# lukors/kanter_core

Measured on AMD Instinct MI355X. Metric: node-Mpix/s on 4096x4096 f32x4, 32-node graph, higher is better.
Workload: dtype f32

## Files before the change

bindings/rust/kanter_core_amd_sys.rs:

```rust
#![allow(non_camel_case_types, dead_code)]
use std::os::raw::{c_char, c_void};

pub const KC_OK: i32 = 0;
pub const KC_ERR_GENERIC: i32 = 1;
pub const KC_ERR_CANCELED: i32 = 2;
pub const KC_ERR_IMAGE: i32 = 3;
pub const KC_ERR_INVALID_BUFFER_COUNT: i32 = 4;
pub const KC_ERR_INVALID_NODE_ID: i32 = 5;
pub const KC_ERR_INVALID_NODE_TYPE: i32 = 6;
pub const KC_ERR_INVALID_SLOT_ID: i32 = 7;
pub const KC_ERR_INVALID_SLOT_TYPE: i32 = 8;
pub const KC_ERR_INVALID_EDGE: i32 = 9;
pub const KC_ERR_NO_SLOT_DATA: i32 = 10;
pub const KC_ERR_SLOT_OCCUPIED: i32 = 11;
pub const KC_ERR_SLOT_NOT_OCCUPIED: i32 = 12;
pub const KC_ERR_UNABLE_TO_LOCK: i32 = 13;
pub const KC_ERR_NODE_PROCESSING: i32 = 14;
pub const KC_ERR_POISON: i32 = 15;
pub const KC_ERR_TRY_LOCK: i32 = 16;
pub const KC_ERR_NODE_DIRTY: i32 = 17;
pub const KC_ERR_IO: i32 = 18;
pub const KC_ERR_INVALID_NAME: i32 = 19;
pub const KC_ERR_HIP: i32 = 100;
pub const KC_ERR_NO_DEVICE: i32 = 101;
// ... 264 lines not shown
    pub fn kc_status_string(status: i32) -> *const c_char;
    pub fn kc_set_fusion(enabled: i32) -> i32;
    pub fn kc_get_fusion() -> i32;
    pub fn kc_set_resize_mode(mode: i32) -> i32;
    pub fn kc_get_resize_mode() -> i32;
    pub fn kc_set_cache_policy(mode: i32) -> i32;
    pub fn kc_get_cache_policy() -> i32;
    pub fn kc_set_option(name: *const c_char, value: i32) -> i32;
    pub fn kc_get_option(name: *const c_char, value: *mut i32) -> i32;
    pub fn kc_resize_upsample_plan(in_n: u32, out_n: u32, filter: i32, eligible: *mut i32, info: *mut i32, rows: *mut f32, cap: usize) -> i32;
    pub fn kc_resize_down2_plan(in_n: u32, out_n: u32, filter: i32, info: *mut i32, left_count: *mut u32, w: *mut f32, wcap: usize, vrec: *mut u32, vcap: usize, hw: *mut f32, hcap: usize) -> i32;
    pub fn kc_stats(bytes_in_use: *mut u64, bytes_cached: *mut u64, kernel_launches: *mut u64) -> i32;
    pub fn kc_stats_algorithmic_bytes(bytes: *mut u64) -> i32;
    pub fn kc_stats_counter(name: *const c_char, value: *mut u64) -> i32;
    pub fn kc_pool_trim() -> i32;
    pub fn kc_set_specialize(mode: i32, after: i32) -> i32;
    pub fn kc_get_specialize() -> i32;
    pub fn kc_specialize_wait() -> i32;
    pub fn kc_specialize_stats(kernels_compiled: *mut u64, compiles_failed: *mut u64, specialized_launches: *mut u64, compiles_pending: *mut u64) -> i32;
    pub fn kc_specialize_compile_check(words: *const u32, n_ops: u32, n_in: u32, start_src: i32, flat: i32, source: *mut c_char, cap: usize) -> i32;
    pub fn kc_specialize_compile_check_mask(words: *const u32, n_ops: u32, n_in: u32, start_src: i32, flat: i32, nt_mask: u32, source: *mut c_char, cap: usize) -> i32;
    pub fn kc_set_chain_quads(quads: i32) -> i32;
    pub fn kc_get_chain_quads() -> i32;
    pub fn kc_specialize_compile_check_upsample(words: *const u32, n_ops: u32, n_in: u32, start_src: i32, taps: u32, wide: i32, source: *mut c_char, cap: usize) -> i32;
    pub fn kc_kernel_cache_set_dir(dir: *const c_char) -> i32;
    pub fn kc_kernel_cache_stats(files_accepted: *mut u64, files_refused: *mut u64, files_written: *mut u64, kernels_loaded: *mut u64) -> i32;
    pub fn kc_kernel_cache_precompile(words: *const u32, n_ops: u32, n_in: u32, start_src: i32, flat: i32, nt_mask: u32, up_taps: u32, up_wide: i32, dir: *const c_char) -> i32;
    pub fn kc_specialize_reset() -> i32;
    pub fn kc_kernel_cache_precompile_packed(words: *const u32, n_ops: u32, n_in: u32, start_src: i32, flat: i32, nt_mask: u32, in_tiers: u32, dir: *const c_char) -> i32;
    pub fn kc_set_pack_sources(mode: i32) -> i32;
    pub fn kc_get_pack_sources() -> i32;
    pub fn kc_set_pack_budget_mb(mb: i32) -> i32;
    pub fn kc_get_pack_budget_mb() -> i32;
    pub fn kc_plane_alloc(width: u32, height: u32, out: *mut *mut KcPlane) -> i32;
    pub fn kc_plane_const(width: u32, height: u32, value: f32, out: *mut *mut KcPlane) -> i32;
    pub fn kc_plane_wrap(device_ptr: *mut c_void, width: u32, height: u32, pitch_bytes: usize, out: *mut *mut KcPlane) -> i32;
    pub fn kc_plane_retain(p: *mut KcPlane) -> i32;
    pub fn kc_plane_release(p: *mut KcPlane) -> i32;
    pub fn kc_plane_size(p: *const KcPlane, width: *mut u32, height: *mut u32) -> i32;
    pub fn kc_plane_is_const(p: *const KcPlane, is_const: *mut i32, value: *mut f32) -> i32;
    pub fn kc_plane_materialize(p: *mut KcPlane) -> i32;
    pub fn kc_plane_device_ptr(p: *mut KcPlane, device_ptr: *mut *mut c_void, pitch_bytes: *mut usize) -> i32;
    pub fn kc_plane_upload_f32(p: *mut KcPlane, host: *const f32, host_pitch_bytes: usize) -> i32;
    pub fn kc_plane_download_f32(p: *mut KcPlane, host: *mut f32, host_pitch_bytes: usize) -> i32;
    pub fn kc_image_gray(p: *mut KcPlane, out: *mut *mut KcImage) -> i32;
    pub fn kc_image_rgba(planes: *const *mut KcPlane, out: *mut *mut KcImage) -> i32;
    pub fn kc_image_retain(img: *mut KcImage) -> i32;
    pub fn kc_image_release(img: *mut KcImage) -> i32;
    pub fn kc_image_is_rgba(img: *const KcImage, is_rgba: *mut i32) -> i32;
    pub fn kc_image_size(img: *const KcImage, size: *mut KcSize) -> i32;
    pub fn kc_image_plane(img: *const KcImage, channel: i32, out: *mut *mut KcPlane) -> i32;
    pub fn kc_image_from_value(size: KcSize, value: f32, rgba: i32, out: *mut *mut KcImage) -> i32;
    pub fn kc_image_as_type(img: *const KcImage, rgba: i32, out: *mut *mut KcImage) -> i32;
    pub fn kc_image_materialize(img: *mut KcImage) -> i32;
    pub fn kc_image_from_u8(host: *const u8, width: u32, height: u32, channels: i32, out: *mut *mut KcImage) -> i32;
    pub fn kc_image_to_u8(img: *mut KcImage, srgb: i32, host_rgba8: *mut u8) -> i32;
    pub fn kc_u8_pipe_create(width: u32, height: u32, channels: i32, depth: i32, out: *mut *mut KcU8Pipe) -> i32;
    pub fn kc_u8_pipe_free(pipe: *mut KcU8Pipe) -> i32;
    pub fn kc_u8_pipe_buffers(pipe: *mut KcU8Pipe, slot: i32, host_in: *mut *mut u8, host_out: *mut *const u8) -> i32;
    pub fn kc_u8_pipe_upload(pipe: *mut KcU8Pipe, slot: i32, out: *mut *mut KcImage) -> i32;
    pub fn kc_u8_pipe_download(pipe: *mut KcU8Pipe, slot: i32, img: *mut KcImage, srgb: i32) -> i32;
    pub fn kc_u8_pipe_wait_download(pipe: *mut KcU8Pipe, slot: i32) -> i32;
    pub fn kc_image_from_f32(host_planes: *const *const f32, n_planes: i32, width: u32, height: u32, out: *mut *mut KcImage) -> i32;
    pub fn kc_image_to_f32(img: *mut KcImage, host_planes: *const *mut f32, n_planes: i32) -> i32;
    pub fn kc_device_image_validate(d: *const KcDeviceImage, extent_bytes: *mut usize) -> i32;
    pub fn kc_image_from_device(src: *const KcDeviceImage, flags: u32, hip_stream: *mut c_void, out: *mut *mut KcImage) -> i32;
// ... 129 lines not shown
```

include/kanter_core_amd.h:

```cpp
#ifndef KANTER_CORE_AMD_H
#define KANTER_CORE_AMD_H

#include <stddef.h>
#include <stdint.h>

#ifdef __cplusplus
extern "C" {
#endif

#define KC_API __attribute__((visibility("default")))

typedef enum kc_status {
    KC_OK = 0,
    KC_ERR_GENERIC = 1,
    KC_ERR_CANCELED = 2,
    KC_ERR_IMAGE = 3,
    KC_ERR_INVALID_BUFFER_COUNT = 4,
    KC_ERR_INVALID_NODE_ID = 5,
    KC_ERR_INVALID_NODE_TYPE = 6,
    KC_ERR_INVALID_SLOT_ID = 7,
    KC_ERR_INVALID_SLOT_TYPE = 8,
    KC_ERR_INVALID_EDGE = 9,
    KC_ERR_NO_SLOT_DATA = 10,
    KC_ERR_SLOT_OCCUPIED = 11,
// ... 66 lines not shown
KC_API int kc_get_option(const char *name, int *value);
KC_API int kc_resize_upsample_plan(uint32_t in_n, uint32_t out_n, int filter, int *eligible, int32_t info[5], float *rows,
                                   size_t cap);
KC_API int kc_resize_down2_plan(uint32_t in_n, uint32_t out_n, int filter, int32_t info[5], uint32_t *left_count, float *w, size_t wcap,
                                uint32_t *vrec, size_t vcap, float *hw, size_t hcap);
KC_API int kc_stats(uint64_t *bytes_in_use, uint64_t *bytes_cached, uint64_t *kernel_launches);
KC_API int kc_stats_algorithmic_bytes(uint64_t *bytes);
KC_API int kc_stats_counter(const char *name, uint64_t *value);
KC_API int kc_pool_trim(void);
KC_API int kc_set_specialize(int mode, int after);
KC_API int kc_get_specialize(void);
KC_API int kc_specialize_wait(void);
KC_API int kc_specialize_stats(uint64_t *kernels_compiled, uint64_t *compiles_failed, uint64_t *specialized_launches,
                               uint64_t *compiles_pending);
KC_API int kc_specialize_compile_check(const uint32_t *words, uint32_t n_ops, uint32_t n_in, int start_src, int flat,
                                       char *source, size_t cap);
KC_API int kc_specialize_compile_check_mask(const uint32_t *words, uint32_t n_ops, uint32_t n_in, int start_src, int flat,
                                            uint32_t nt_mask, char *source, size_t cap);
KC_API int kc_set_chain_quads(int quads);
KC_API int kc_get_chain_quads(void);
KC_API int kc_specialize_compile_check_upsample(const uint32_t *words, uint32_t n_ops, uint32_t n_in, int start_src, uint32_t taps,
                                                int wide, char *source, size_t cap);
KC_API int kc_kernel_cache_set_dir(const char *dir);
KC_API int kc_kernel_cache_stats(uint64_t *files_accepted, uint64_t *files_refused, uint64_t *files_written, uint64_t *kernels_loaded);
KC_API int kc_kernel_cache_precompile(const uint32_t *words, uint32_t n_ops, uint32_t n_in, int start_src, int flat, uint32_t nt_mask,
                                      uint32_t up_taps, int up_wide, const char *dir);
KC_API int kc_specialize_reset(void);
KC_API int kc_kernel_cache_precompile_packed(const uint32_t *words, uint32_t n_ops, uint32_t n_in, int start_src, int flat,
                                             uint32_t nt_mask, uint32_t in_tiers, const char *dir);
KC_API int kc_set_pack_sources(int mode);
KC_API int kc_get_pack_sources(void);
KC_API int kc_set_pack_budget_mb(int mb);
KC_API int kc_get_pack_budget_mb(void);

KC_API int kc_plane_alloc(uint32_t width, uint32_t height, kc_plane **out);
KC_API int kc_plane_const(uint32_t width, uint32_t height, float value, kc_plane **out);
KC_API int kc_plane_wrap(void *device_ptr, uint32_t width, uint32_t height, size_t pitch_bytes, kc_plane **out);
KC_API int kc_plane_retain(kc_plane *p);
KC_API int kc_plane_release(kc_plane *p);
KC_API int kc_plane_size(const kc_plane *p, uint32_t *width, uint32_t *height);
KC_API int kc_plane_is_const(const kc_plane *p, int *is_const, float *value);
KC_API int kc_plane_materialize(kc_plane *p);
KC_API int kc_plane_device_ptr(kc_plane *p, void **device_ptr, size_t *pitch_bytes);
KC_API int kc_plane_upload_f32(kc_plane *p, const float *host, size_t host_pitch_bytes);
KC_API int kc_plane_download_f32(kc_plane *p, float *host, size_t host_pitch_bytes);

KC_API int kc_image_gray(kc_plane *p, kc_image **out);
KC_API int kc_image_rgba(kc_plane *const planes[4], kc_image **out);
KC_API int kc_image_retain(kc_image *img);
KC_API int kc_image_release(kc_image *img);
KC_API int kc_image_is_rgba(const kc_image *img, int *is_rgba);
KC_API int kc_image_size(const kc_image *img, kc_size *size);
KC_API int kc_image_plane(const kc_image *img, int channel, kc_plane **out);
KC_API int kc_image_from_value(kc_size size, float value, int rgba, kc_image **out);
KC_API int kc_image_as_type(const kc_image *img, int rgba, kc_image **out);
KC_API int kc_image_materialize(kc_image *img);
KC_API int kc_image_from_u8(const uint8_t *host, uint32_t width, uint32_t height, int channels, kc_image **out);
KC_API int kc_image_to_u8(kc_image *img, int srgb, uint8_t *host_rgba8);
KC_API int kc_u8_pipe_create(uint32_t width, uint32_t height, int channels, int depth, kc_u8_pipe **out);
KC_API int kc_u8_pipe_free(kc_u8_pipe *pipe);
KC_API int kc_u8_pipe_buffers(kc_u8_pipe *pipe, int slot, uint8_t **host_in, const uint8_t **host_out);
KC_API int kc_u8_pipe_upload(kc_u8_pipe *pipe, int slot, kc_image **out);
KC_API int kc_u8_pipe_download(kc_u8_pipe *pipe, int slot, kc_image *img, int srgb);
KC_API int kc_u8_pipe_wait_download(kc_u8_pipe *pipe, int slot);
KC_API int kc_image_from_f32(const float *const host_planes[], int n_planes, uint32_t width, uint32_t height, kc_image **out);
KC_API int kc_image_to_f32(kc_image *img, float *const host_planes[], int n_planes);
// ... 253 lines not shown
```

kanter_core_amd/__init__.py:

```python
from .api import (Edge, EmbeddedSlotDataId, LiveGraph, MixType, Node, NodeGraph, NodeId, NodeState, NodeType,
                  ResizeFilter, ResizePolicy, Side, Size, SlotData, SlotId, SlotImage, TexProError,
                  TextureProcessor, calculate_size, combine_rgba_process, get_stream, height_to_normal_process,
                  init, is_initialized, mix_process, resize_image, separate_rgba_process, set_fusion, set_stream,
                  shutdown, stats, sync, value_process, set_specialize, get_specialize, specialize_wait,
                  specialize_stats, specialize_compile_check, Partition, PartitionPolicy, NodeKind, set_resize_mode,
                  get_resize_mode, resize_upsample_plan, resize_down2_plan, stats_counter, specialize_compile_check_upsample, specialize_compile_check_mask, set_chain_quads, get_chain_quads, set_pack_sources, get_pack_sources, set_pack_budget_mb, get_pack_budget_mb, set_cache_policy, get_cache_policy, set_option, get_option, comm_unique_id, comm_init,
                  comm_destroy, comm_info, comm_stats, comm_transport, comm_gather_bands, PlanKind, pool_trim, kernel_cache_set_dir, kernel_cache_stats,
                  kernel_cache_precompile, specialize_reset, U8Pipe, device_image_desc, DEVICE_SRGB, DEVICE_GRAY,
                  ChannelStats, STATS_HISTOGRAM, STATS_SRGB, BC_SRGB, BC6H, BC7, BC_BLOCK_BYTES,
                  MIP_PER_LEVEL, MIP_NORMALS, MIP_COVERAGE, MIP_ALPHA_WEIGHT, mip_alpha_weight, mip_alpha_texel, mip_coverage_ref, MipCoverageLevel, alpha_ref_threshold, mip_coverage_target, mip_coverage_scale, mip_normal_texel, mip_unit_normal, mip_roughness_texel, levels_to_bc_mips, write_dds_levels, mip_level_count, bc_mip_layout, dds_header, BC_GRAY, BC_ALL_MODES, BcError, DdsInfo, dds_parse, preview_level,
                  PREVIEW_SRGB, PreviewPlan, preview_plan, previews, previews_torch)

__all__ = [n for n in dir() if not n.startswith("_")]
```

kanter_core_amd/_abi.py:

```python
import ctypes as C


KC_OK = 0
KC_ERR_GENERIC = 1
KC_ERR_CANCELED = 2
KC_ERR_IMAGE = 3
KC_ERR_INVALID_BUFFER_COUNT = 4
KC_ERR_INVALID_NODE_ID = 5
KC_ERR_INVALID_NODE_TYPE = 6
KC_ERR_INVALID_SLOT_ID = 7
KC_ERR_INVALID_SLOT_TYPE = 8
KC_ERR_INVALID_EDGE = 9
KC_ERR_NO_SLOT_DATA = 10
KC_ERR_SLOT_OCCUPIED = 11
KC_ERR_SLOT_NOT_OCCUPIED = 12
KC_ERR_UNABLE_TO_LOCK = 13
KC_ERR_NODE_PROCESSING = 14
KC_ERR_POISON = 15
KC_ERR_TRY_LOCK = 16
KC_ERR_NODE_DIRTY = 17
KC_ERR_IO = 18
KC_ERR_INVALID_NAME = 19
KC_ERR_HIP = 100
KC_ERR_NO_DEVICE = 101
# ... 285 lines not shown
    "kc_status_string": (C.c_char_p, [C.c_int]),
    "kc_set_fusion": (C.c_int, [C.c_int]),
    "kc_get_fusion": (C.c_int, []),
    "kc_set_resize_mode": (C.c_int, [C.c_int]),
    "kc_get_resize_mode": (C.c_int, []),
    "kc_set_cache_policy": (C.c_int, [C.c_int]),
    "kc_get_cache_policy": (C.c_int, []),
    "kc_set_option": (C.c_int, [C.c_char_p, C.c_int]),
    "kc_get_option": (C.c_int, [C.c_char_p, C.POINTER(C.c_int)]),
    "kc_resize_upsample_plan": (C.c_int, [C.c_uint32, C.c_uint32, C.c_int, C.POINTER(C.c_int), C.POINTER(C.c_int32), C.c_void_p, C.c_size_t]),
    "kc_resize_down2_plan": (C.c_int, [C.c_uint32, C.c_uint32, C.c_int, C.POINTER(C.c_int32), C.POINTER(C.c_uint32), C.c_void_p, C.c_size_t, C.POINTER(C.c_uint32), C.c_size_t, C.c_void_p, C.c_size_t]),
    "kc_stats": (C.c_int, [C.POINTER(C.c_uint64), C.POINTER(C.c_uint64), C.POINTER(C.c_uint64)]),
    "kc_stats_algorithmic_bytes": (C.c_int, [C.POINTER(C.c_uint64)]),
    "kc_stats_counter": (C.c_int, [C.c_char_p, C.POINTER(C.c_uint64)]),
    "kc_pool_trim": (C.c_int, []),
    "kc_set_specialize": (C.c_int, [C.c_int, C.c_int]),
    "kc_get_specialize": (C.c_int, []),
    "kc_specialize_wait": (C.c_int, []),
    "kc_specialize_stats": (C.c_int, [C.POINTER(C.c_uint64), C.POINTER(C.c_uint64), C.POINTER(C.c_uint64), C.POINTER(C.c_uint64)]),
    "kc_specialize_compile_check": (C.c_int, [C.POINTER(C.c_uint32), C.c_uint32, C.c_uint32, C.c_int, C.c_int, C.c_char_p, C.c_size_t]),
    "kc_specialize_compile_check_mask": (C.c_int, [C.POINTER(C.c_uint32), C.c_uint32, C.c_uint32, C.c_int, C.c_int, C.c_uint32, C.c_char_p, C.c_size_t]),
    "kc_set_chain_quads": (C.c_int, [C.c_int]),
    "kc_get_chain_quads": (C.c_int, []),
    "kc_specialize_compile_check_upsample": (C.c_int, [C.POINTER(C.c_uint32), C.c_uint32, C.c_uint32, C.c_int, C.c_uint32, C.c_int, C.c_char_p, C.c_size_t]),
    "kc_kernel_cache_set_dir": (C.c_int, [C.c_char_p]),
    "kc_kernel_cache_stats": (C.c_int, [C.POINTER(C.c_uint64), C.POINTER(C.c_uint64), C.POINTER(C.c_uint64), C.POINTER(C.c_uint64)]),
    "kc_kernel_cache_precompile": (C.c_int, [C.POINTER(C.c_uint32), C.c_uint32, C.c_uint32, C.c_int, C.c_int, C.c_uint32, C.c_uint32, C.c_int, C.c_char_p]),
    "kc_specialize_reset": (C.c_int, []),
    "kc_kernel_cache_precompile_packed": (C.c_int, [C.POINTER(C.c_uint32), C.c_uint32, C.c_uint32, C.c_int, C.c_int, C.c_uint32, C.c_uint32, C.c_char_p]),
    "kc_set_pack_sources": (C.c_int, [C.c_int]),
    "kc_get_pack_sources": (C.c_int, []),
    "kc_set_pack_budget_mb": (C.c_int, [C.c_int]),
    "kc_get_pack_budget_mb": (C.c_int, []),
    "kc_plane_alloc": (C.c_int, [C.c_uint32, C.c_uint32, C.POINTER(C.c_void_p)]),
    "kc_plane_const": (C.c_int, [C.c_uint32, C.c_uint32, C.c_float, C.POINTER(C.c_void_p)]),
    "kc_plane_wrap": (C.c_int, [C.c_void_p, C.c_uint32, C.c_uint32, C.c_size_t, C.POINTER(C.c_void_p)]),
    "kc_plane_retain": (C.c_int, [C.c_void_p]),
    "kc_plane_release": (C.c_int, [C.c_void_p]),
    "kc_plane_size": (C.c_int, [C.c_void_p, C.POINTER(C.c_uint32), C.POINTER(C.c_uint32)]),
    "kc_plane_is_const": (C.c_int, [C.c_void_p, C.POINTER(C.c_int), C.c_void_p]),
    "kc_plane_materialize": (C.c_int, [C.c_void_p]),
    "kc_plane_device_ptr": (C.c_int, [C.c_void_p, C.POINTER(C.c_void_p), C.POINTER(C.c_size_t)]),
    "kc_plane_upload_f32": (C.c_int, [C.c_void_p, C.c_void_p, C.c_size_t]),
    "kc_plane_download_f32": (C.c_int, [C.c_void_p, C.c_void_p, C.c_size_t]),
    "kc_image_gray": (C.c_int, [C.c_void_p, C.POINTER(C.c_void_p)]),
    "kc_image_rgba": (C.c_int, [C.POINTER(C.c_void_p), C.POINTER(C.c_void_p)]),
    "kc_image_retain": (C.c_int, [C.c_void_p]),
    "kc_image_release": (C.c_int, [C.c_void_p]),
    "kc_image_is_rgba": (C.c_int, [C.c_void_p, C.POINTER(C.c_int)]),
    "kc_image_size": (C.c_int, [C.c_void_p, C.POINTER(kc_size)]),
    "kc_image_plane": (C.c_int, [C.c_void_p, C.c_int, C.POINTER(C.c_void_p)]),
    "kc_image_from_value": (C.c_int, [kc_size, C.c_float, C.c_int, C.POINTER(C.c_void_p)]),
    "kc_image_as_type": (C.c_int, [C.c_void_p, C.c_int, C.POINTER(C.c_void_p)]),
    "kc_image_materialize": (C.c_int, [C.c_void_p]),
    "kc_image_from_u8": (C.c_int, [C.c_void_p, C.c_uint32, C.c_uint32, C.c_int, C.POINTER(C.c_void_p)]),
    "kc_image_to_u8": (C.c_int, [C.c_void_p, C.c_int, C.c_void_p]),
    "kc_u8_pipe_create": (C.c_int, [C.c_uint32, C.c_uint32, C.c_int, C.c_int, C.POINTER(C.c_void_p)]),
    "kc_u8_pipe_free": (C.c_int, [C.c_void_p]),
    "kc_u8_pipe_buffers": (C.c_int, [C.c_void_p, C.c_int, C.POINTER(C.c_void_p), C.POINTER(C.c_void_p)]),
    "kc_u8_pipe_upload": (C.c_int, [C.c_void_p, C.c_int, C.POINTER(C.c_void_p)]),
    "kc_u8_pipe_download": (C.c_int, [C.c_void_p, C.c_int, C.c_void_p, C.c_int]),
    "kc_u8_pipe_wait_download": (C.c_int, [C.c_void_p, C.c_int]),
    "kc_image_from_f32": (C.c_int, [C.POINTER(C.c_void_p), C.c_int, C.c_uint32, C.c_uint32, C.POINTER(C.c_void_p)]),
    "kc_image_to_f32": (C.c_int, [C.c_void_p, C.POINTER(C.c_void_p), C.c_int]),
    "kc_device_image_validate": (C.c_int, [C.POINTER(kc_device_image), C.POINTER(C.c_size_t)]),
    "kc_image_from_device": (C.c_int, [C.POINTER(kc_device_image), C.c_uint32, C.c_void_p, C.POINTER(C.c_void_p)]),
# ... 129 lines not shown
```

kanter_core_amd/api.py:

```python
import collections
import ctypes as C
import os

import numpy as np

from . import _abi, _lib
from ._lib import kc_edge, kc_node_desc, kc_size

_VARIANT_NAMES = {"KC_ERR_POISON": "PoisonError", "KC_ERR_TRY_LOCK": "TryLockError", "KC_ERR_INVALID_ARG": "InvalidArgument"}
_ERROR_NAMES = {v: _VARIANT_NAMES.get(k, k[len("KC_ERR_"):].title().replace("_", ""))
                for k, v in vars(_abi).items() if k.startswith("KC_ERR_")}


class TexProError(Exception):

    def __init__(self, code, detail=""):
        self.code = code
        self.kind = _ERROR_NAMES.get(code, "Unknown")
        L = _lib.load()
        msg = L.kc_status_string(code).decode()
        super().__init__("%s: %s%s" % (self.kind, msg, (" (" + detail + ")") if detail else ""))

    def __eq__(self, other):
        return isinstance(other, TexProError) and other.code == self.code
# ... 172 lines not shown
    return buf.value.decode()


def specialize_compile_check_mask(words, n_in, nt_mask, start_src=0, flat=True):
    arr = (C.c_uint32 * len(words))(*words)
    buf = C.create_string_buffer(1 << 17)
    _check(_lib.load().kc_specialize_compile_check_mask(arr, len(words), int(n_in), int(start_src), int(bool(flat)), int(nt_mask),
                                                        buf, len(buf)))
    return buf.value.decode()


def set_chain_quads(quads):
    _check(_lib.load().kc_set_chain_quads(int(quads)))


def get_chain_quads():
    return _lib.load().kc_get_chain_quads()


def set_pack_sources(mode):
    _check(_lib.load().kc_set_pack_sources(int(mode)))


def get_pack_sources():
    return _lib.load().kc_get_pack_sources()


def set_pack_budget_mb(mb):
    _check(_lib.load().kc_set_pack_budget_mb(int(mb)))


def get_pack_budget_mb():
    return _lib.load().kc_get_pack_budget_mb()


def specialize_compile_check_upsample(words, n_in, start_src=0, taps=3, wide=True):
    arr = (C.c_uint32 * len(words))(*words)
    buf = C.create_string_buffer(1 << 17)
    _check(_lib.load().kc_specialize_compile_check_upsample(arr, len(words), int(n_in), int(start_src), int(taps), int(bool(wide)),
                                                            buf, len(buf)))
    return buf.value.decode()


def stats():
    a, b, c = C.c_uint64(), C.c_uint64(), C.c_uint64()
    _check(_lib.load().kc_stats(C.byref(a), C.byref(b), C.byref(c)))
    d = C.c_uint64()
    _check(_lib.load().kc_stats_algorithmic_bytes(C.byref(d)))
    return {"bytes_in_use": a.value, "bytes_cached": b.value, "kernel_launches": c.value, "algorithmic_bytes": d.value}


def kernel_cache_set_dir(path):
    _check(_lib.load().kc_kernel_cache_set_dir(None if path is None else str(path).encode()))


def kernel_cache_stats():
    v = [C.c_uint64() for _ in range(4)]
    _check(_lib.load().kc_kernel_cache_stats(*[C.byref(x) for x in v]))
    return dict(zip(("files_accepted", "files_refused", "files_written", "kernels_loaded"), (x.value for x in v)))


def kernel_cache_precompile(words, n_in, start_src, flat, nt_mask, directory, up_taps=0, up_wide=False, in_tiers=0):
    arr = (C.c_uint32 * len(words))(*words)
    if in_tiers:
        if up_taps:
            raise ValueError("packed inputs: plain chain programs only")
# ... 1397 lines not shown
```

kanter_core_amd/csrc/c_api.cpp:

```cpp
#include <algorithm>
#include <cctype>
#include <climits>
#include <cstdio>
#include <cstdlib>
#include <cstring>
#include <fstream>
#include <sstream>

#include "kc_runtime.hpp"

namespace kc {
const std::string &last_error();
}
using namespace kc;

#define KC_ARG(cond)                                         \
    do {                                                     \
        if (!(cond)) {                                       \
            set_error("invalid argument: " #cond);           \
            return KC_ERR_INVALID_ARG;                       \
        }                                                    \
    } while (0)

typedef std::lock_guard<std::recursive_mutex> Lock;
// ... 417 lines not shown
KC_CATCH

int kc_kernel_cache_precompile_packed(const uint32_t *words, uint32_t n_ops, uint32_t n_in, int start_src, int flat, uint32_t nt_mask,
                                      uint32_t in_tiers, const char *dir)
try {
    KC_ARG(words && dir);
    std::string log = "in_tiers: two bits per input plane, 0 to 2, flat programs only";
    const int s = kernel_cache_precompile(words, n_ops, n_in, start_src, flat != 0, nt_mask, in_tiers, 0, false, dir, &log);
    if (s != KC_OK) set_error("kernel cache: " + log);
    return s;
}
KC_CATCH

int kc_set_pack_sources(int mode)
try {
    Lock lk(ctx().mu);
    if (mode < 0 || mode > 2) {
        set_error("kc_set_pack_sources accepts 0, 1 or 2");
        return KC_ERR_INVALID_ARG;
    }
    ctx().pack_sources = mode;
    return KC_OK;
}
KC_CATCH

int kc_get_pack_sources(void)
try {
    return ctx().pack_sources;
}
catch (...) {
    return 0;
}

int kc_set_pack_budget_mb(int mb)
try {
    Lock lk(ctx().mu);
    if (mb < 0) {
        set_error("kc_set_pack_budget_mb accepts 0 and up");
        return KC_ERR_INVALID_ARG;
    }
    ctx().pack_budget_mb = mb;
    return KC_OK;
}
KC_CATCH

int kc_get_pack_budget_mb(void)
try {
    return ctx().pack_budget_mb;
}
catch (...) {
    return 0;
}

int kc_specialize_reset(void)
try {
    Lock lk(ctx().mu);
    if (ctx().stream) (void)hipStreamSynchronize(ctx().stream);
    const int mode = specialize_get_mode();
    specialize_shutdown();
    (void)mode;
    return KC_OK;
}
KC_CATCH

int kc_specialize_compile_check_upsample(const uint32_t *words, uint32_t n_ops, uint32_t n_in, int start_src, uint32_t taps, int wide,
                                         char *source, size_t cap)
// ... 1558 lines not shown
```

kanter_core_amd/csrc/chain_pack.cpp:

```cpp
#include "kc_runtime.hpp"

namespace kc {

uint32_t pack_bytes_per_quad(uint32_t tier) { return tier == (uint32_t)KC_PACK_FIX24 ? 12u : tier == (uint32_t)KC_PACK_U8 ? 4u : 16u; }

void plane_shadow_drop(kc_plane *p, bool never_again)
{
    if (p->shadow) {
        Context &c = ctx();
        pool_free(p->shadow, p->shadow_bytes);
        c.shadow_bytes -= p->shadow_bytes;
        c.counters["packed_bytes"] = c.shadow_bytes;
        p->shadow = nullptr;
        p->shadow_bytes = 0;
    }
    p->pack_tier = KC_PACK_NONE;
    p->pack_seen = 0;
    p->pack_state = never_again ? kc_plane::PACK_NEVER : kc_plane::PACK_UNTRIED;
}

static bool plane_packable(const kc_plane *p, uint32_t w, uint32_t h)
{
    return p && p->kind == kc_plane::MEM && p->owned && !p->view_of && p->dptr && p->w == w && p->h == h && w % 4 == 0 &&
           (p->pitch == (size_t)w * 4 || h == 1) && p->pack_state != kc_plane::PACK_NEVER;
}

static size_t shadow_block(uint64_t quads, uint32_t tier) { return (size_t)((quads * pack_bytes_per_quad(tier) + 255) / 256 * 256); }

static void pack_slot(kc_plane *const *planes, int n)
{
    Context &c = ctx();
    const uint64_t quads = (uint64_t)planes[0]->w * planes[0]->h / 4;
    const uint64_t budget = (uint64_t)c.pack_budget_mb << 20;
    if (c.shadow_bytes + (uint64_t)n * shadow_block(quads, KC_PACK_U8) > budget) return;
    static const uint32_t kTiers[2] = { KC_PACK_U8, KC_PACK_FIX24 };
    void *blk[KC_CHAIN_MAX_BATCH][2] = {};
    PoolStaging flags;
    uint32_t host[KC_CHAIN_MAX_BATCH][2];
    bool ok = flags.alloc(sizeof host) == KC_OK && hipMemsetAsync(flags.ptr, 0, sizeof host, c.stream) == hipSuccess;
    for (int i = 0; i < n && ok; ++i)
        for (int t = 0; t < 2 && ok; ++t) {
            ok = pool_alloc(shadow_block(quads, kTiers[t]), &blk[i][t]) == KC_OK &&
                 launch_pack_plane(kTiers[t], planes[i]->dptr, blk[i][t], quads, (uint32_t *)flags.ptr + 2 * i + t, c.stream) == hipSuccess;
        }
    ok = ok && hipMemcpyAsync(host, flags.ptr, sizeof host, hipMemcpyDeviceToHost, c.stream) == hipSuccess;
    ok = hipStreamSynchronize(c.stream) == hipSuccess && ok;
    c.counters["pack_passes"] += 2 * (uint64_t)n;
    c.alg_bytes += (uint64_t)n * quads * (16 + 4 + 16 + 12);
    int keep = -1;
    for (int t = 0; t < 2 && ok && keep < 0; ++t) {
        bool all = true;
        for (int i = 0; i < n; ++i) all = all && host[i][t] == 0;
        if (all) keep = t;
    }
    if (!ok) (void)hipGetLastError();
    if (ok && keep < 0) c.counters["pack_rejected"] += (uint64_t)n;
    if (keep >= 0 && c.shadow_bytes + (uint64_t)n * shadow_block(quads, kTiers[keep]) > budget) keep = -1;
    for (int i = 0; i < n; ++i) {
        for (int t = 0; t < 2; ++t)
            if (blk[i][t] && t != keep) pool_free(blk[i][t], shadow_block(quads, kTiers[t]));
        kc_plane *p = planes[i];
        if (keep < 0) {
            p->pack_state = kc_plane::PACK_NEVER;
            continue;
        }
        p->shadow = blk[i][keep];
        p->shadow_bytes = shadow_block(quads, kTiers[keep]);
        p->pack_tier = (uint8_t)kTiers[keep];
        p->pack_state = kc_plane::PACKED;
        c.shadow_bytes += p->shadow_bytes;
        c.counters["packed_planes"]++;
    }
    c.counters["packed_bytes"] = c.shadow_bytes;
}

uint32_t pack_chain_inputs(const ChainProgram &P, int batch, kc_plane *const (*src)[KC_CHAIN_MAX_IN], const uint32_t *refs, uint32_t w, uint32_t h)
{
    Context &c = ctx();
    const int mode = c.pack_sources;
    if (!mode || !src || !refs || batch < 1 || batch > (int)KC_CHAIN_MAX_BATCH) return 0;
    const uint64_t px4 = 4ull * w * h * (uint64_t)batch;
    if (mode == 1 && (uint64_t)P.n_in * px4 + px4 <= ((uint64_t)c.opt.cache_budget_mb << 20)) return 0;
    struct Slot {
        kc_plane *todo[KC_CHAIN_MAX_BATCH];
        int n_todo = 0;
        bool ok = false;
    } slots[KC_CHAIN_MAX_IN];
    bool due = true;
    for (uint32_t k = 0; k < P.n_in; ++k) {
        Slot &sl = slots[k];
        if (refs[k] < 2) continue;
        sl.ok = true;
        for (int b = 0; b < batch && sl.ok; ++b) {
            kc_plane *p = src[b][k];
            sl.ok = plane_packable(p, w, h) && (const float *)p->dptr == P.in[b][k];
            if (!sl.ok || p->pack_state == kc_plane::PACKED) continue;
            bool seen = false;
            for (int i = 0; i < sl.n_todo; ++i) seen = seen || sl.todo[i] == p;
            if (seen) continue;
            sl.todo[sl.n_todo++] = p;
            if (p->pack_seen < 255) ++p->pack_seen;
            if (mode == 1 && p->pack_seen < 2) due = false;
        }
    }
    if (!due) return 0;
    uint32_t tiers = 0;
    for (uint32_t k = 0; k < P.n_in; ++k) {
        Slot &sl = slots[k];
        if (!sl.ok) continue;
        if (sl.n_todo) pack_slot(sl.todo, sl.n_todo);
        uint32_t tier = src[0][k]->pack_state == kc_plane::PACKED ? src[0][k]->pack_tier : 0u;
        for (int b = 1; b < batch; ++b)
            if (src[b][k]->pack_state != kc_plane::PACKED || src[b][k]->pack_tier != tier) tier = 0;
        tiers |= tier << (2 * k);
    }
    return tiers;
}

}
```

kanter_core_amd/csrc/kc_runtime.hpp:

```cpp
#pragma once

#include <cstring>
#include <deque>
#include <set>
#include <tuple>
#include <type_traits>
#include <unordered_map>
#include <unordered_set>

#include "kc_internal.hpp"

namespace kc {
struct Chain;
struct ChainLink;
}

namespace kc {
#if defined(__SANITIZE_ADDRESS__) || defined(__SANITIZE_THREAD__)
#define KC_NO_OBJECT_POOL 1
#elif defined(__has_feature)
#if __has_feature(address_sanitizer) || __has_feature(thread_sanitizer)
#define KC_NO_OBJECT_POOL 1
#endif
#endif
// ... 362 lines not shown
int preview_check(const kc_preview_request *r, uint32_t count, uint32_t flags, const void *out, size_t out_bytes, bool images_named, const char *who);
int image_previews(const kc_preview_request *r, kc_image *const *imgs, uint32_t count, uint32_t flags, uint8_t *host, size_t host_bytes, const char *who);
int image_previews_device(const kc_preview_request *r, uint32_t count, uint32_t flags, void *device_ptr, size_t bytes, void *hip_stream);
void preview_release();
int image_channel_stats(kc_image *img, uint32_t flags, kc_channel_stats *out);
uint32_t quant_u8_host(float v);
int stats_buffers(size_t partials_bytes);
void channel_stats_release();
int calculate_size(int policy, const kc_size *sizes, int n, int slot_index, kc_size specific, kc_size *out);
int mix_process(kc_image *left, kc_image *right, int mix_type, kc_image **out);
int separate_process(kc_image *in, kc_image *out[4]);
int combine_process(kc_image *const in[4], kc_image **out);
int value_process(float v, kc_image **out);
int height_to_normal_process(kc_image *in, kc_image **out);
int height_to_normal_band(kc_image *in_with_halo, uint32_t full_h, kc_image **out);

int build_taps_host(uint32_t in_n, uint32_t out_n, int filter, TapsHost &t);
int resize_image(kc_image *src, kc_size size, int filter, kc_image **out);
int resize_force(kc_plane *p);
int resize_planes_band(kc_plane *const *srcs, int n, int32_t src_y0, uint32_t src_h_full, kc_size dst_full, int32_t a, int32_t b,
                       int filter, kc_plane **outs);
int resize_force_many(kc_plane *const *planes, int n);
int chain_resize_launch(const ChainProgram &P, int batch, int mode, kc_plane *const *sampled, bool *launched);

hipError_t launch_chain_specialized(const ChainProgram &P, int batch, hipStream_t s, bool *launched, uint32_t *nt_mask, uint32_t *quads = nullptr);
uint32_t cache_policy_mask(uint64_t in_bytes, uint64_t out_bytes, uint32_t n_resident, const Options &o = options());
uint32_t chain_cache_policy(const uint32_t *refs, uint32_t n, uint64_t stream_bytes, uint64_t out_bytes);
hipError_t chain_dispatch(ChainProgram &P, int batch, int mode, uint32_t w, uint32_t h, size_t out_pitch_bytes,
                          kc_plane *const (*src)[KC_CHAIN_MAX_IN] = nullptr, const uint32_t *refs = nullptr, uint64_t *packed_saved = nullptr);
uint32_t pack_chain_inputs(const ChainProgram &P, int batch, kc_plane *const (*src)[KC_CHAIN_MAX_IN], const uint32_t *refs, uint32_t w, uint32_t h);
void plane_shadow_drop(kc_plane *p, bool never_again);
uint32_t pack_bytes_per_quad(uint32_t tier);
bool chain_pack_program_ok(const ChainProgram &P);
hipError_t launch_upsample_chain_specialized(const ChainProgram &P, int batch, const UpsampleArgs &U, hipStream_t s, bool *launched);
int specialize_set_mode(int mode, int after);
int specialize_get_mode();
int specialize_set_chain_quads(int quads);
int specialize_get_chain_quads();
void specialize_wait();
void specialize_stats(uint64_t *compiled, uint64_t *failed, uint64_t *launches, uint64_t *pending);
std::string specialize_last_log();
void specialize_shutdown();
std::string specialize_source(const ChainProgram &P, const UpsampleArgs *U = nullptr);
int specialize_compile_only(const ChainProgram &P, std::string *log, const UpsampleArgs *U = nullptr);
int kernel_cache_set_dir(const char *dir);
void kernel_cache_stats(uint64_t *hits, uint64_t *rejected, uint64_t *written, uint64_t *kernels_loaded);
bool kernel_cache_populated();
int kernel_cache_precompile(const uint32_t *words, uint32_t n_ops, uint32_t n_in, int32_t start_src, bool flat, uint32_t nt_mask, uint32_t in_tiers,
                            uint32_t up_taps, bool up_wide, const char *dir, std::string *log);

int u8_pipe_create(uint32_t w, uint32_t h, int channels, int depth, kc_u8_pipe **out);
int u8_pipe_free(kc_u8_pipe *p);
int u8_pipe_buffers(kc_u8_pipe *p, int slot, uint8_t **host_in, const uint8_t **host_out);
int u8_pipe_upload(kc_u8_pipe *p, int slot, kc_image **out);
int u8_pipe_download(kc_u8_pipe *p, int slot, kc_image *img, bool srgb);
int u8_pipe_wait_download(kc_u8_pipe *p, int slot);

int png_read(const std::string &path, std::vector<uint8_t> &px, uint32_t &w, uint32_t &h, int &channels);
int png_write_rgba8(const std::string &path, const uint8_t *px, uint32_t w, uint32_t h);

struct NodeGraph;

struct Node {
    uint32_t node_id = 0;
    int type = KC_NODE_VALUE;
    int mix_type = KC_MIX_ADD;
// ... 248 lines not shown
```

kanter_core_amd/csrc/specialize.cpp:

```cpp
#include <dlfcn.h>
#include <sys/stat.h>
#include <unistd.h>

#include <condition_variable>
#include <cstdio>
#include <cstdlib>
#include <cstring>
#include <thread>

#include "kc_runtime.hpp"

namespace kc {

extern const char kJitChainProgramH[];
extern const char kJitPowPositiveInc[];
extern const char kJitUpsampleH[];
extern const char kJitUpsampleChainInc[];
extern const char kJitChainPackH[] __attribute__((weak));

namespace {

typedef struct _hiprtcProgram *hiprtcProgram;
struct Rtc {
    void *lib = nullptr;
// ... 60 lines not shown
        k.append((const char *)&nt_mask, sizeof nt_mask);
        k.append((const char *)word, sizeof(uint32_t) * n_ops);
        if (quads > 1) {
            k.push_back('q');
            k.push_back((char)('0' + quads));
        }
        if (in_tiers) {
            k.push_back('t');
            k.append((const char *)&in_tiers, sizeof in_tiers);
        }
        return k;
    }
};

constexpr uint32_t kQuadsWarm = 2, kQuadsMaxOps = 16;
std::atomic<int> g_chain_quads{ 0 };

uint32_t chain_quads_for(const Signature &s, uint64_t total_units)
{
    if (s.up_taps || !s.flat || s.n_in < 1 || s.n_ops > kQuadsMaxOps || total_units > 0xF0000000ull) return 1;
    bool plain = false;
    for (uint32_t k = 0; k < s.n_in; ++k) plain |= !(s.nt_mask & KC_CHAIN_NT_BIT(k));
    if (!plain || !s.nt_mask) return 1;
    for (uint32_t i = 0; i < s.n_ops; ++i) {
        const uint32_t code = s.word[i] & 0xffu;
        if (code == CH_DIV_L || code == CH_DIV_R || code == CH_POW_L || code == CH_POW_R) return 1;
    }
    const int forced = g_chain_quads.load(std::memory_order_relaxed);
    return forced ? (uint32_t)forced : kQuadsWarm;
}

bool pack_program_ok(const ChainProgram &P)
{
    if (P.n_ops < 1 || P.n_ops > kQuadsMaxOps || P.n_in < 1 || P.rows != 1) return false;
    for (uint32_t i = 0; i < P.n_ops; ++i) {
        const uint32_t code = ((i & 1u) ? P.step[0][i / 2].b.word : P.step[0][i / 2].a.word) & 0xffu;
        if (code == CH_DIV_L || code == CH_DIV_R || code == CH_POW_L || code == CH_POW_R) return false;
    }
    return true;
}

Signature signature_of(const ChainProgram &P, const UpsampleArgs *U = nullptr)
{
    Signature s;
    s.n_in = P.n_in;
    s.n_ops = P.n_ops;
    s.start_src = P.start_src;
    s.flat = U ? false : P.rows == 1;
    {
        uint32_t valid = 0x100u;
        for (uint32_t k = 0; k < (U ? P.n_in - 1u : P.n_in); ++k) valid |= KC_CHAIN_NT_BIT(k);
        s.nt_mask = P.nt_mask & valid;
    }
    if (U) {
        s.up_taps = U->H.taps;
        s.up_wide = U->tile_w == 1024;
    }
    for (uint32_t i = 0; i < P.n_ops; ++i) s.word[i] = (i & 1u) ? P.step[0][i / 2].b.word : P.step[0][i / 2].a.word;
    if (!U && s.flat) s.in_tiers = P.n_in >= 16 ? P.in_tiers : P.in_tiers & ((1u << (2 * P.n_in)) - 1u);
    s.quads = chain_quads_for(s, (uint64_t)P.rows * P.row_units);
    return s;
}

static int spec_wg()
{
    static int wg = [] {
        int v = 256;
        if (const char *e = std::getenv("KC_SPEC_WG")) {
            const int x = std::atoi(e);
            if (x == 64 || x == 128 || x == 256 || x == 512 || x == 1024) v = x;
        }
        return v;
// ... 715 lines not shown
    }
    lk.unlock();
    S.cv.notify_one();
    return nullptr;
}

hipError_t launch_chain_specialized(const ChainProgram &P, int batch, hipStream_t s, bool *launched, uint32_t *nt_mask, uint32_t *quads)
{
    *launched = false;
    if (P.n_ops < 1 || P.n_ops > (uint32_t)KC_CHAIN_MAX_OPS || P.n_in > (uint32_t)KC_CHAIN_MAX_IN) return hipSuccess;
    const uint64_t total = (uint64_t)P.rows * P.row_units;
    if (total == 0 || total > 0xFFFFFFFFull) return hipSuccess;
    const Signature sig = signature_of(P);
    hipFunction_t fn = spec_lookup(sig);
    if (!fn) return hipSuccess;
    size_t size = sizeof(ChainProgram);
    const int SPEC_WG = spec_wg();
    void *extra[] = { HIP_LAUNCH_PARAM_BUFFER_POINTER, (void *)&P, HIP_LAUNCH_PARAM_BUFFER_SIZE, &size, HIP_LAUNCH_PARAM_END };
    const uint64_t per_block = (uint64_t)SPEC_WG * sig.quads;
    const unsigned gx = (unsigned)((total + per_block - 1) / per_block);
    hipError_t e = hipModuleLaunchKernel(fn, gx, (unsigned)batch, 1, SPEC_WG, 1, 1, 0, s, nullptr, extra);
    if (e == hipSuccess) {
        *launched = true;
        if (nt_mask) *nt_mask = sig.nt_mask;
        if (quads) *quads = sig.quads;
        std::lock_guard<std::mutex> lk(spec().mu);
        spec().launches++;
    }
    return e;
}

bool chain_pack_program_ok(const ChainProgram &P) { return pack_program_ok(P); }

hipError_t launch_upsample_chain_specialized(const ChainProgram &P, int batch, const UpsampleArgs &U, hipStream_t s, bool *launched)
{
    *launched = false;
    if (P.n_ops < 1 || P.n_ops > (uint32_t)KC_CHAIN_MAX_OPS || P.n_in < 1 || P.n_in > (uint32_t)KC_CHAIN_INTERP_IN) return hipSuccess;
    if (!upsample_args_ok(U, batch) || (U.H.taps != 1 && U.H.taps != 3)) return hipSuccess;
    if (U.H.ratio == 2) return hipSuccess;
    hipFunction_t fn = spec_lookup(signature_of(P, &U));
    if (!fn) return hipSuccess;
    struct alignas(16) Params {
        ChainProgram P;
        UpsampleArgs U;
    };
    static_assert(sizeof(ChainProgram) % alignof(UpsampleArgs) == 0, "the second kernel argument follows the first without padding");
    static thread_local Params params;
    params.P = P;
    params.U = U;
    size_t size = sizeof(Params);
    void *extra[] = { HIP_LAUNCH_PARAM_BUFFER_POINTER, (void *)&params, HIP_LAUNCH_PARAM_BUFFER_SIZE, &size, HIP_LAUNCH_PARAM_END };
    const dim3 grid = upsample_grid(U, batch);
    hipError_t e = hipModuleLaunchKernel(fn, grid.x, grid.y, grid.z, 256, 1, 1, (unsigned)upsample_lds_bytes(U), s, nullptr, extra);
    if (e == hipSuccess) {
        *launched = true;
        std::lock_guard<std::mutex> lk(spec().mu);
        spec().launches++;
    }
    return e;
}

int specialize_set_mode(int mode, int after)
{
    Spec &S = spec();
    if (mode < 0 || mode > 2) return KC_ERR_INVALID_ARG;
    {
// ... 154 lines not shown
```

Baseline: 7.144 million.

## Batch source packing into one sync and gate packed launches by a cost model

Packing of several chain inputs is grouped so that one stream synchronize and one flag copy cover many slots, where before each slot needed its own. A roofline-style cost rule compares estimated VALU issue time with memory-byte time and only allows packed-source launches when the chain stays bandwidth-bound. The op-count limit on packing is dropped in favour of this rule. This should cut host sync overhead and avoid packing where decode ALU work would dominate, at the cost of hardcoded throughput constants that may misjudge some chains.

```diff
diff --git a/bindings/rust/kanter_core_amd_sys.rs b/bindings/rust/kanter_core_amd_sys.rs
--- a/bindings/rust/kanter_core_amd_sys.rs
+++ b/bindings/rust/kanter_core_amd_sys.rs
@@ -320,6 +320,7 @@
     pub fn kc_get_pack_sources() -> i32;
     pub fn kc_set_pack_budget_mb(mb: i32) -> i32;
     pub fn kc_get_pack_budget_mb() -> i32;
+    pub fn kc_pack_cost_rule(words: *const u32, n_ops: u32, n_in: u32, in_tiers: u32, quads: u32, units: u64, packs: *mut i32, issue_ns: *mut f64, bytes_ns: *mut f64) -> i32;
     pub fn kc_plane_alloc(width: u32, height: u32, out: *mut *mut KcPlane) -> i32;
     pub fn kc_plane_const(width: u32, height: u32, value: f32, out: *mut *mut KcPlane) -> i32;
     pub fn kc_plane_wrap(device_ptr: *mut c_void, width: u32, height: u32, pitch_bytes: usize, out: *mut *mut KcPlane) -> i32;
diff --git a/include/kanter_core_amd.h b/include/kanter_core_amd.h
--- a/include/kanter_core_amd.h
+++ b/include/kanter_core_amd.h
@@ -122,6 +122,8 @@
 KC_API int kc_get_pack_sources(void);
 KC_API int kc_set_pack_budget_mb(int mb);
 KC_API int kc_get_pack_budget_mb(void);
+KC_API int kc_pack_cost_rule(const uint32_t *words, uint32_t n_ops, uint32_t n_in, uint32_t in_tiers, uint32_t quads, uint64_t units,
+                             int *packs, double *issue_ns, double *bytes_ns);
 
 KC_API int kc_plane_alloc(uint32_t width, uint32_t height, kc_plane **out);
 KC_API int kc_plane_const(uint32_t width, uint32_t height, float value, kc_plane **out);
diff --git a/kanter_core_amd/__init__.py b/kanter_core_amd/__init__.py
--- a/kanter_core_amd/__init__.py
+++ b/kanter_core_amd/__init__.py
@@ -4,7 +4,7 @@
                   init, is_initialized, mix_process, resize_image, separate_rgba_process, set_fusion, set_stream,
                   shutdown, stats, sync, value_process, set_specialize, get_specialize, specialize_wait,
                   specialize_stats, specialize_compile_check, Partition, PartitionPolicy, NodeKind, set_resize_mode,
-                  get_resize_mode, resize_upsample_plan, resize_down2_plan, stats_counter, specialize_compile_check_upsample, specialize_compile_check_mask, set_chain_quads, get_chain_quads, set_pack_sources, get_pack_sources, set_pack_budget_mb, get_pack_budget_mb, set_cache_policy, get_cache_policy, set_option, get_option, comm_unique_id, comm_init,
+                  get_resize_mode, resize_upsample_plan, resize_down2_plan, stats_counter, specialize_compile_check_upsample, specialize_compile_check_mask, set_chain_quads, get_chain_quads, set_pack_sources, get_pack_sources, pack_cost_rule, set_pack_budget_mb, get_pack_budget_mb, set_cache_policy, get_cache_policy, set_option, get_option, comm_unique_id, comm_init,
                   comm_destroy, comm_info, comm_stats, comm_transport, comm_gather_bands, PlanKind, pool_trim, kernel_cache_set_dir, kernel_cache_stats,
                   kernel_cache_precompile, specialize_reset, U8Pipe, device_image_desc, DEVICE_SRGB, DEVICE_GRAY,
                   ChannelStats, STATS_HISTOGRAM, STATS_SRGB, BC_SRGB, BC6H, BC7, BC_BLOCK_BYTES,
diff --git a/kanter_core_amd/_abi.py b/kanter_core_amd/_abi.py
--- a/kanter_core_amd/_abi.py
+++ b/kanter_core_amd/_abi.py
@@ -341,6 +341,7 @@
     "kc_get_pack_sources": (C.c_int, []),
     "kc_set_pack_budget_mb": (C.c_int, [C.c_int]),
     "kc_get_pack_budget_mb": (C.c_int, []),
+    "kc_pack_cost_rule": (C.c_int, [C.POINTER(C.c_uint32), C.c_uint32, C.c_uint32, C.c_uint32, C.c_uint32, C.c_uint64, C.POINTER(C.c_int), C.POINTER(C.c_double), C.POINTER(C.c_double)]),
     "kc_plane_alloc": (C.c_int, [C.c_uint32, C.c_uint32, C.POINTER(C.c_void_p)]),
     "kc_plane_const": (C.c_int, [C.c_uint32, C.c_uint32, C.c_float, C.POINTER(C.c_void_p)]),
     "kc_plane_wrap": (C.c_int, [C.c_void_p, C.c_uint32, C.c_uint32, C.c_size_t, C.POINTER(C.c_void_p)]),
diff --git a/kanter_core_amd/api.py b/kanter_core_amd/api.py
--- a/kanter_core_amd/api.py
+++ b/kanter_core_amd/api.py
@@ -228,6 +228,14 @@
 
 def get_pack_budget_mb():
     return _lib.load().kc_get_pack_budget_mb()
+
+
+def pack_cost_rule(words, n_in, in_tiers, quads=1, units=1 << 20):
+    arr = (C.c_uint32 * len(words))(*words)
+    packs, issue, mem = C.c_int(), C.c_double(), C.c_double()
+    _check(_lib.load().kc_pack_cost_rule(arr, len(words), int(n_in), int(in_tiers), int(quads), int(units), C.byref(packs),
+                                         C.byref(issue), C.byref(mem)))
+    return bool(packs.value), issue.value, mem.value
 
 
 def specialize_compile_check_upsample(words, n_in, start_src=0, taps=3, wide=True):
diff --git a/kanter_core_amd/csrc/c_api.cpp b/kanter_core_amd/csrc/c_api.cpp
--- a/kanter_core_amd/csrc/c_api.cpp
+++ b/kanter_core_amd/csrc/c_api.cpp
@@ -473,6 +473,17 @@
     return 0;
 }
 
+int kc_pack_cost_rule(const uint32_t *words, uint32_t n_ops, uint32_t n_in, uint32_t in_tiers, uint32_t quads, uint64_t units, int *packs,
+                      double *issue_ns, double *bytes_ns)
+try {
+    KC_ARG(words && packs && n_ops >= 1 && n_ops <= (uint32_t)KC_CHAIN_MAX_OPS && n_in >= 1 && n_in <= (uint32_t)KC_CHAIN_MAX_IN);
+    KC_ARG(quads == 1 || quads == 2 || quads == 4);
+    for (uint32_t k = 0; k < 16; ++k) KC_ARG(KC_CHAIN_TIER(in_tiers, k) != 3u && (k < n_in || KC_CHAIN_TIER(in_tiers, k) == 0u));
+    *packs = chain_pack_cost_ok(words, n_ops, n_in, in_tiers, quads, units, issue_ns, bytes_ns) ? 1 : 0;
+    return KC_OK;
+}
+KC_CATCH
+
 int kc_set_pack_budget_mb(int mb)
 try {
     Lock lk(ctx().mu);
diff --git a/kanter_core_amd/csrc/chain_pack.cpp b/kanter_core_amd/csrc/chain_pack.cpp
--- a/kanter_core_amd/csrc/chain_pack.cpp
+++ b/kanter_core_amd/csrc/chain_pack.cpp
@@ -27,49 +27,67 @@
 
 static size_t shadow_block(uint64_t quads, uint32_t tier) { return (size_t)((quads * pack_bytes_per_quad(tier) + 255) / 256 * 256); }
 
-static void pack_slot(kc_plane *const *planes, int n)
+static const uint32_t kTiers[2] = { KC_PACK_U8, KC_PACK_FIX24 };
+
+struct PackSlot {
+    kc_plane *todo[KC_CHAIN_MAX_BATCH];
+    int n_todo = 0;
+    bool ok = false;
+    void *blk[KC_CHAIN_MAX_BATCH][2] = {};
+};
+
+static uint64_t slot_pass_bytes(const PackSlot &sl, uint64_t quads)
+{
+    return (uint64_t)sl.n_todo * (shadow_block(quads, KC_PACK_U8) + shadow_block(quads, KC_PACK_FIX24));
+}
+
+static void pack_slots(PackSlot *slots, uint32_t first, uint32_t last, uint64_t quads)
 {
     Context &c = ctx();
-    const uint64_t quads = (uint64_t)planes[0]->w * planes[0]->h / 4;
     const uint64_t budget = (uint64_t)c.pack_budget_mb << 20;
-    if (c.shadow_bytes + (uint64_t)n * shadow_block(quads, KC_PACK_U8) > budget) return;
-    static const uint32_t kTiers[2] = { KC_PACK_U8, KC_PACK_FIX24 };
-    void *blk[KC_CHAIN_MAX_BATCH][2] = {};
     PoolStaging flags;
-    uint32_t host[KC_CHAIN_MAX_BATCH][2];
+    uint32_t host[KC_CHAIN_MAX_IN][KC_CHAIN_MAX_BATCH][2];
     bool ok = flags.alloc(sizeof host) == KC_OK && hipMemsetAsync(flags.ptr, 0, sizeof host, c.stream) == hipSuccess;
-    for (int i = 0; i < n && ok; ++i)
-        for (int t = 0; t < 2 && ok; ++t) {
-            ok = pool_alloc(shadow_block(quads, kTiers[t]), &blk[i][t]) == KC_OK &&
-                 launch_pack_plane(kTiers[t], planes[i]->dptr, blk[i][t], quads, (uint32_t *)flags.ptr + 2 * i + t, c.stream) == hipSuccess;
-        }
+    for (uint32_t k = first; k < last && ok; ++k)
+        for (int i = 0; i < slots[k].n_todo && ok; ++i)
+            for (int t = 0; t < 2 && ok; ++t) {
+                uint32_t *flag = (uint32_t *)flags.ptr + ((size_t)k * KC_CHAIN_MAX_BATCH + i) * 2 + t;
+                ok = pool_alloc(shadow_block(quads, kTiers[t]), &slots[k].blk[i][t]) == KC_OK &&
+                     launch_pack_plane(kTiers[t], slots[k].todo[i]->dptr, slots[k].blk[i][t], quads, flag, c.stream) == hipSuccess;
+            }
     ok = ok && hipMemcpyAsync(host, flags.ptr, sizeof host, hipMemcpyDeviceToHost, c.stream) == hipSuccess;
     ok = hipStreamSynchronize(c.stream) == hipSuccess && ok;
-    c.counters["pack_passes"] += 2 * (uint64_t)n;
-    c.alg_bytes += (uint64_t)n * quads * (16 + 4 + 16 + 12);
-    int keep = -1;
-    for (int t = 0; t < 2 && ok && keep < 0; ++t) {
-        bool all = true;
-        for (int i = 0; i < n; ++i) all = all && host[i][t] == 0;
-        if (all) keep = t;
-    }
+    c.counters["pack_syncs"]++;
     if (!ok) (void)hipGetLastError();
-    if (ok && keep < 0) c.counters["pack_rejected"] += (uint64_t)n;
-    if (keep >= 0 && c.shadow_bytes + (uint64_t)n * shadow_block(quads, kTiers[keep]) > budget) keep = -1;
-    for (int i = 0; i < n; ++i) {
-        for (int t = 0; t < 2; ++t)
-            if (blk[i][t] && t != keep) pool_free(blk[i][t], shadow_block(quads, kTiers[t]));
-        kc_plane *p = planes[i];
-        if (keep < 0) {
-            p->pack_state = kc_plane::PACK_NEVER;
-            continue;
+    for (uint32_t k = first; k < last; ++k) {
+        PackSlot &sl = slots[k];
+        const int n = sl.n_todo;
+        if (!n) continue;
+        c.counters["pack_passes"] += 2 * (uint64_t)n;
+        c.alg_bytes += (uint64_t)n * quads * (16 + 4 + 16 + 12);
+        int keep = -1;
+        for (int t = 0; t < 2 && ok && keep < 0; ++t) {
+            bool all = true;
+            for (int i = 0; i < n; ++i) all = all && host[k][i][t] == 0;
+            if (all) keep = t;
         }
-        p->shadow = blk[i][keep];
-        p->shadow_bytes = shadow_block(quads, kTiers[keep]);
-        p->pack_tier = (uint8_t)kTiers[keep];
-        p->pack_state = kc_plane::PACKED;
-        c.shadow_bytes += p->shadow_bytes;
-        c.counters["packed_planes"]++;
+        if (ok && keep < 0) c.counters["pack_rejected"] += (uint64_t)n;
+        if (keep >= 0 && c.shadow_bytes + (uint64_t)n * shadow_block(quads, kTiers[keep]) > budget) keep = -1;
+        for (int i = 0; i < n; ++i) {
+            for (int t = 0; t < 2; ++t)
+                if (sl.blk[i][t] && t != keep) pool_free(sl.blk[i][t], shadow_block(quads, kTiers[t]));
+            kc_plane *p = sl.todo[i];
+            if (keep < 0) {
+                p->pack_state = kc_plane::PACK_NEVER;
+                continue;
+            }
+            p->shadow = sl.blk[i][keep];
+            p->shadow_bytes = shadow_block(quads, kTiers[keep]);
+            p->pack_tier = (uint8_t)kTiers[keep];
+            p->pack_state = kc_plane::PACKED;
+            c.shadow_bytes += p->shadow_bytes;
+            c.counters["packed_planes"]++;
+        }
     }
     c.counters["packed_bytes"] = c.shadow_bytes;
 }
@@ -81,14 +99,10 @@
     if (!mode || !src || !refs || batch < 1 || batch > (int)KC_CHAIN_MAX_BATCH) return 0;
     const uint64_t px4 = 4ull * w * h * (uint64_t)batch;
     if (mode == 1 && (uint64_t)P.n_in * px4 + px4 <= ((uint64_t)c.opt.cache_budget_mb << 20)) return 0;
-    struct Slot {
-        kc_plane *todo[KC_CHAIN_MAX_BATCH];
-        int n_todo = 0;
-        bool ok = false;
-    } slots[KC_CHAIN_MAX_IN];
+    PackSlot slots[KC_CHAIN_MAX_IN];
     bool due = true;
     for (uint32_t k = 0; k < P.n_in; ++k) {
-        Slot &sl = slots[k];
+        PackSlot &sl = slots[k];
         if (refs[k] < 2) continue;
         sl.ok = true;
         for (int b = 0; b < batch && sl.ok; ++b) {
@@ -96,7 +110,8 @@
             sl.ok = plane_packable(p, w, h) && (const float *)p->dptr == P.in[b][k];
             if (!sl.ok || p->pack_state == kc_plane::PACKED) continue;
             bool seen = false;
-            for (int i = 0; i < sl.n_todo; ++i) seen = seen || sl.todo[i] == p;
+            for (uint32_t j = 0; j <= k; ++j)
+                for (int i = 0; i < slots[j].n_todo; ++i) seen = seen || slots[j].todo[i] == p;
             if (seen) continue;
             sl.todo[sl.n_todo++] = p;
             if (p->pack_seen < 255) ++p->pack_seen;
@@ -104,16 +119,43 @@
         }
     }
     if (!due) return 0;
+    if (mode == 1) {
+        uint32_t maybe = 0;
+        for (uint32_t k = 0; k < P.n_in; ++k)
+            if (slots[k].ok) maybe |= (slots[k].n_todo ? (uint32_t)KC_PACK_FIX24 : (uint32_t)src[0][k]->pack_tier) << (2 * k);
+        if (!maybe || !chain_pack_launch_ok(P, batch, maybe)) return 0;
+    }
+    {
+        const uint64_t quads = (uint64_t)w * h / 4, budget = (uint64_t)c.pack_budget_mb << 20;
+        uint32_t first = 0;
+        uint64_t group = 0;
+        for (uint32_t k = 0; k < P.n_in; ++k) {
+            PackSlot &sl = slots[k];
+            if (!sl.ok || !sl.n_todo) continue;
+            if (group && c.shadow_bytes + group + slot_pass_bytes(sl, quads) > budget) {
+                pack_slots(slots, first, k, quads);
+                group = 0;
+            }
+            if (!group) {
+                if (c.shadow_bytes + (uint64_t)sl.n_todo * shadow_block(quads, KC_PACK_U8) > budget) {
+                    sl.n_todo = 0;
+                    continue;
+                }
+                first = k;
+            }
+            group += slot_pass_bytes(sl, quads);
+        }
+        if (group) pack_slots(slots, first, P.n_in, quads);
+    }
     uint32_t tiers = 0;
     for (uint32_t k = 0; k < P.n_in; ++k) {
-        Slot &sl = slots[k];
-        if (!sl.ok) continue;
-        if (sl.n_todo) pack_slot(sl.todo, sl.n_todo);
+        if (!slots[k].ok) continue;
         uint32_t tier = src[0][k]->pack_state == kc_plane::PACKED ? src[0][k]->pack_tier : 0u;
         for (int b = 1; b < batch; ++b)
             if (src[b][k]->pack_state != kc_plane::PACKED || src[b][k]->pack_tier != tier) tier = 0;
         tiers |= tier << (2 * k);
     }
+    if (mode == 1 && tiers && !chain_pack_launch_ok(P, batch, tiers)) return 0;
     return tiers;
 }
 
diff --git a/kanter_core_amd/csrc/kc_runtime.hpp b/kanter_core_amd/csrc/kc_runtime.hpp
--- a/kanter_core_amd/csrc/kc_runtime.hpp
+++ b/kanter_core_amd/csrc/kc_runtime.hpp
@@ -418,6 +418,9 @@
 void plane_shadow_drop(kc_plane *p, bool never_again);
 uint32_t pack_bytes_per_quad(uint32_t tier);
 bool chain_pack_program_ok(const ChainProgram &P);
+bool chain_pack_cost_ok(const uint32_t *words, uint32_t n_ops, uint32_t n_in, uint32_t in_tiers, uint32_t quads, uint64_t units, double *issue_ns,
+                        double *bytes_ns);
+bool chain_pack_launch_ok(const ChainProgram &P, int batch, uint32_t in_tiers);
 hipError_t launch_upsample_chain_specialized(const ChainProgram &P, int batch, const UpsampleArgs &U, hipStream_t s, bool *launched);
 int specialize_set_mode(int mode, int after);
 int specialize_get_mode();
diff --git a/kanter_core_amd/csrc/specialize.cpp b/kanter_core_amd/csrc/specialize.cpp
--- a/kanter_core_amd/csrc/specialize.cpp
+++ b/kanter_core_amd/csrc/specialize.cpp
@@ -116,12 +116,36 @@
 
 bool pack_program_ok(const ChainProgram &P)
 {
-    if (P.n_ops < 1 || P.n_ops > kQuadsMaxOps || P.n_in < 1 || P.rows != 1) return false;
+    if (P.n_ops < 1 || P.n_in < 1 || P.rows != 1) return false;
     for (uint32_t i = 0; i < P.n_ops; ++i) {
         const uint32_t code = ((i & 1u) ? P.step[0][i / 2].b.word : P.step[0][i / 2].a.word) & 0xffu;
         if (code == CH_DIV_L || code == CH_DIV_R || code == CH_POW_L || code == CH_POW_R) return false;
     }
     return true;
+}
+
+constexpr double kIssueNsPerInst = 1.97, kPackBytesPerNs = 6100.0, kPackIssueShare = 0.75;
+constexpr uint32_t kQuadValu = 5, kDecodeValuFix24 = 12, kDecodeValuU8 = 10, kSimds = 1024, kWaveLanes = 64;
+
+bool pack_cost_ok(const uint32_t *words, uint32_t n_ops, uint32_t n_in, uint32_t in_tiers, uint32_t quads, uint64_t units, double *issue_ns,
+                  double *bytes_ns)
+{
+    uint32_t valu = kQuadValu + n_in, bytes = 16;
+    for (uint32_t i = 0; i < n_ops; ++i) {
+        const uint32_t code = words[i] & 0xffu;
+        valu += code == CH_SAVE_LOAD ? 0u : code == CH_ADD_INV || code == CH_SUBL_INV || code == CH_SUBR_INV || code == CH_MUL_INV ? 4u : 2u;
+    }
+    for (uint32_t k = 0; k < n_in; ++k) {
+        const uint32_t tier = KC_CHAIN_TIER(in_tiers, k);
+        valu += tier == (uint32_t)KC_PACK_FIX24 ? kDecodeValuFix24 : tier == (uint32_t)KC_PACK_U8 ? kDecodeValuU8 : 0u;
+        bytes += tier == (uint32_t)KC_PACK_FIX24 ? 12u : tier == (uint32_t)KC_PACK_U8 ? 4u : 16u;
+    }
+    if (quads < 1) quads = 1;
+    const double waves_per_simd = (double)units / (double)(kWaveLanes * quads) / (double)kSimds;
+    const double issue = waves_per_simd * (double)(valu * quads) * kIssueNsPerInst, mem = (double)units * (double)bytes / kPackBytesPerNs;
+    if (issue_ns) *issue_ns = issue;
+    if (bytes_ns) *bytes_ns = mem;
+    return issue <= kPackIssueShare * mem;
 }
 
 Signature signature_of(const ChainProgram &P, const UpsampleArgs *U = nullptr)
@@ -903,6 +927,19 @@
 
 bool chain_pack_program_ok(const ChainProgram &P) { return pack_program_ok(P); }
 
+bool chain_pack_cost_ok(const uint32_t *words, uint32_t n_ops, uint32_t n_in, uint32_t in_tiers, uint32_t quads, uint64_t units, double *issue_ns,
+                        double *bytes_ns)
+{
+    return pack_cost_ok(words, n_ops, n_in, in_tiers, quads, units, issue_ns, bytes_ns);
+}
+
+bool chain_pack_launch_ok(const ChainProgram &P, int batch, uint32_t in_tiers)
+{
+    if (P.n_ops > (uint32_t)KC_CHAIN_MAX_OPS || P.n_in > (uint32_t)KC_CHAIN_MAX_IN) return false;
+    const Signature s = signature_of(P);
+    return pack_cost_ok(s.word, s.n_ops, s.n_in, in_tiers, s.quads, (uint64_t)P.rows * P.row_units * (uint64_t)batch, nullptr, nullptr);
+}
+
 hipError_t launch_upsample_chain_specialized(const ChainProgram &P, int batch, const UpsampleArgs &U, hipStream_t s, bool *launched)
 {
     *launched = false;
```

After: 7.071 million. -1.0%, worse.
